# janelia-flyem/transfer_em

Hardware: AMD Instinct MI355X
Metric: CycleGAN train steps/sec on 132^3 x1 uint8 volumes (per-GPU batch of 1 volume; aggregate over GPUs) (higher is better)
Workload: dtype f32; 1 GPU; 3D 132^3 single-channel synthetic volumes, batch=1 per GPU, fp32, EM2EM.train_step (BASELINE.json configs[1]); global_batch=1, dimsize=132, parallelism=dp1

## Files before the change

transfer_em_amd/csrc/wino.hip:

```cpp
#include "tem_common.h"
#include "wino_common.h"
#include <cmath>
#include <cstdio>
#include <cstdlib>

namespace wino {

#ifdef TEM_DEBUG_KNOBS
#define KDBG(x) (x)
#else
#define KDBG(x) 0
#endif


struct Ep32 {
  float slope;
  const float *gate; int32_t gN, gD, gH, gW; float gate_slope;
  const uint8_t *keep_mask;
  int32_t doz, doy, dox, dD, dH, dW;
  int32_t gbytes, mbytes;
};

struct Dev {
  const float *in0, *in1;
  int32_t i0N, i0D, i0H, i0W, i1N, i1D, i1H, i1W;
  int32_t C0;
  int32_t N, D, H, W;
  const float *u;
  float *out0, *out1;
  int32_t o0N, o0D, o0H, o0W, o1N, o1D, o1H, o1W;
  int32_t CO0;
  int32_t OD, OH, OW;
  int32_t P;
  int32_t BY, BX, nby, nbx, zsegs, zper, NTZ;
  int32_t E, PLC, subb, slotb;
  int32_t ndma;
  int32_t span0, span1;
  uint32_t magicBX, magicE;
  int32_t dbg;
  int32_t obytes;
  unsigned long long *stamps;
  Ep32 ep;
};

template <int CI, int CO, int NI, int EP, int EE>
__global__ __launch_bounds__(512) void wino_conv_k(Dev p) {
  constexpr int NH = CI / 8, VB = 32;
  constexpr int NB = (CO + 15) / 16;
  constexpr bool STREAM = CI == 32;
  constexpr bool PAIR = CI == 8 && CO == 8;
  constexpr int NKZ = PAIR ? 4 : 3;
  constexpr int UCH = 2 * NB * 16 * 128;
  extern __shared__ __attribute__((aligned(16))) float lds[];
  char *const ring = reinterpret_cast<char *>(lds);
  const int tid = threadIdx.x, lane = tid & 63;
  const int wave = __builtin_amdgcn_readfirstlane(tid >> 6);
  const int m = lane & 15, q = lane >> 4;
  const int grp = PAIR ? wave : (NB == 1 ? wave >> 1 : wave >> 2);
  const int nb = NB == 1 ? 0 : (wave >> 1) & 1;
  const int zb = PAIR ? (q >> 1) : (wave & 1);
  const int co = PAIR ? 4 * (q & 1) : nb * 16 + 4 * q;
  float *const uld = reinterpret_cast<float *>(ring + 4 * p.slotb);

  int seg = (int)xcd_contiguous_block(blockIdx.x, gridDim.x);
  const int zseg = seg % p.zsegs; seg /= p.zsegs;
  const int bx = seg % p.nbx; seg /= p.nbx;
  const int by = seg % p.nby;
  const int n = seg / p.nby;
  const int tz0 = zseg * p.zper, tz1 = min(p.NTZ, tz0 + p.zper), nsteps = tz1 - tz0;
  const int oy0 = by * 2 * p.BY, ox0 = bx * 2 * p.BX;
  const int ntile = p.BY * p.BX;

  const bool two_in = p.in1 != p.in0;
  const float *const in0n = p.in0 + (size_t)n * p.i0N, *const in1n = p.in1 + (size_t)n * p.i1N;
  int voff0[NI], voff1[NI];
  {
    const int iy0 = oy0 - p.P, ix0 = ox0 - p.P;
#pragma unroll
    for (int i = 0; i < NI; ++i) {
      const int sp = (wave + 8 * i) * 64 + lane;
      const bool ex = sp < p.PLC;
      const int spc = ex ? sp : 0;
      const int cpos = spc & 1, ve = spc >> 1;
      const int ro = ve / EE, e = ve - ro * EE;
      const int o = ro & 1, yr = ro >> 1;
      const int c = (cpos ^ swz(e, yr)) * 4;
      const int iy = iy0 + yr, ix = ix0 + 2 * e + o;
      const bool ok = ex && (unsigned)iy < (unsigned)p.H && (unsigned)ix < (unsigned)p.W;
      voff0[i] = ok ? (iy * p.i0H + ix * p.i0W + c) * 4 : (int)0x80000000;
      voff1[i] = ok ? (iy * p.i1H + ix * p.i1W + c) * 4 : (int)0x80000000;
      asm volatile("" : "+v"(voff0[i]), "+v"(voff1[i]));
    }
  }
  auto dma_plane = [&](int iz, int slot) {
    const bool zok = (unsigned)iz < (unsigned)p.D;
    const int izc = zok ? iz : 0;
#pragma unroll
    for (int h = 0; h < NH; ++h) {
      char *const dst = ring + slot * p.slotb + h * p.subb;
      if (!two_in || 8 * h < p.C0)
        dma_subimage<NI, !STREAM>(in0n + izc * p.i0D + 8 * h, zok ? p.span0 - 32 * h : 0, voff0, dst, wave, p.ndma);
      else
        dma_subimage<NI, !STREAM>(in1n + izc * p.i1D + (8 * h - p.C0), zok ? p.span1 - 4 * (8 * h - p.C0) : 0, voff1, dst, wave, p.ndma);
    }
  };

  const int izb0 = 2 * tz0 - p.P;
  if (nsteps > 0) {
#pragma unroll
    for (int k = 0; k < 4; ++k) dma_plane(izb0 + k, k);
  }
  auto dma_u = [&](int chunk, int buf) {
    const __amdgpu_buffer_rsrc_t r = __builtin_amdgcn_make_buffer_rsrc((void *)(p.u + (size_t)chunk * UCH), 0, UCH * 4, 0x00020000);
#pragma unroll
    for (int i = 0; i < UCH * 4 / 1024 / 8; ++i) {
      const int j = wave + 8 * i;
      __builtin_amdgcn_raw_ptr_buffer_load_lds(r, (__attribute__((address_space(3))) void *)((char *)uld + buf * (UCH * 4) + j * 1024), 16,
                                               (j * 64 + lane) * 16, 0, 0, 0);
    }
  };
  if (STREAM) {
    dma_u(0, 0);
  } else {
    constexpr int UF4 = NKZ * NH * NB * 16 * 64 * 2 / 4;
    static_assert(UF4 % 512 == 0, "whole 1 KB wave transfers");
    const __amdgpu_buffer_rsrc_t ur = __builtin_amdgcn_make_buffer_rsrc((void *)p.u, 0, UF4 * 16, 0x00020000);
#pragma unroll
    for (int i = 0; i < UF4 / 512; ++i) {
      const int j = wave + 8 * i;
      __builtin_amdgcn_raw_ptr_buffer_load_lds(ur, (__attribute__((address_space(3))) void *)((char *)uld + j * 1024), 16,
                                               (j * 64 + lane) * 16, 0, 0, 0);
    }
  }
  asm volatile("s_waitcnt vmcnt(0)" ::: "memory");
  __syncthreads();

  constexpr int rowb = EE * VB;
  const Ep32 &ep = p.ep;
  float *const out0n = p.out0 + (size_t)n * p.o0N, *const out1n = EP == 2 ? p.out1 + (size_t)n * p.o1N : nullptr;
  const float *const gaten = EP >= 1 ? ep.gate + (size_t)n * ep.gN : nullptr;
  const bool in0c = EP != 2 || co < p.CO0;
  float *const obase = EP == 2 ? (in0c ? out0n : out1n) : out0n;
  const int oco = in0c ? co : co - p.CO0;
  const int oD = in0c ? p.o0D : p.o1D, oH = in0c ? p.o0H : p.o1H, oW = in0c ? p.o0W : p.o1W;
  const __amdgpu_buffer_rsrc_t grs = __builtin_amdgcn_make_buffer_rsrc((void *)gaten, 0, EP >= 1 ? ep.gbytes : 0, 0x00020000);
  const __amdgpu_buffer_rsrc_t mrs = __builtin_amdgcn_make_buffer_rsrc((void *)ep.keep_mask, 0, EP == 2 ? ep.mbytes : 0, 0x00020000);
  const int mpv = EP == 2 ? p.CO0 >> 3 : 0;
  const int kshift = co & 4;
  int gso[4], mso[4], oso[4];
#pragma unroll
  for (int o4 = 0; o4 < 4; ++o4) {
    gso[o4] = EP >= 1 ? ((o4 >> 1) * ep.gH + (o4 & 1) * ep.gW) * 4 : 0;
    mso[o4] = EP == 2 ? ((o4 >> 1) * ep.dW + (o4 & 1)) * mpv : 0;
    oso[o4] = ((o4 >> 1) * p.o0H + (o4 & 1) * p.o0W) * 4;
  }
  const __amdgpu_buffer_rsrc_t ors = __builtin_amdgcn_make_buffer_rsrc((void *)out0n, 0, EP != 2 ? p.obytes : 0, 0x00020000);

  const int tA = min(grp * 16 + m, ntile - 1);
  const int tyA = (int)fdiv((uint32_t)tA, (uint32_t)p.BX, p.magicBX), txA = tA - tyA * p.BX;
  const int a0 = (4 * tyA * EE + txA) * VB + (q & 1) * 8;
  int cs[2][2];
#pragma unroll
  for (int a = 0; a < 2; ++a)
#pragma unroll
    for (int b = 0; b < 2; ++b) cs[a][b] = ((q >> 1) ^ swz(txA + a, 2 * (tyA + b))) * 16;

#ifdef TEM_DEBUG_KNOBS
  unsigned long long t_last = p.stamps ? clock64() : 0, t_sum[8] = {0, 0, 0, 0, 0, 0, 0, 0};
#define STAMP(i) do { if (p.stamps) { unsigned long long t_now = clock64(); t_sum[i] += t_now - t_last; t_last = t_now; } } while (0)
#else
#define STAMP(i) do { } while (0)
#endif
  f32x4 acc[16];
  f32x4 gv[4];
  uint32_t kb[4];
  uint32_t tyx, tok4 = 0;
  {
    const int t = grp * 16 + m;
    const int ty = (int)fdiv((uint32_t)t, (uint32_t)p.BX, p.magicBX), tx = t - ty * p.BX;
    const int oy = oy0 + 2 * ty, ox = ox0 + 2 * tx;
    const bool tok = co < CO && t < ntile;
#pragma unroll
    for (int o4 = 0; o4 < 4; ++o4) tok4 |= ((tok && oy + (o4 >> 1) < p.OH && ox + (o4 & 1) < p.OW) ? 1u : 0u) << o4;
    tyx = ((uint32_t)oy << 16) | (uint32_t)ox;
  }
  auto tile_geom = [&](int oz, int &o0, int &go, int &mb, uint32_t &okm) {
    uint32_t yx = tyx;
    asm volatile("" : "+v"(yx));
    const int oy = (int)(yx >> 16), ox = (int)(yx & 0xffffu);
    okm = oz < p.OD ? tok4 : 0u;
    o0 = oz * oD + oy * oH + ox * oW + oco;
    go = EP >= 1 ? (oz * ep.gD + oy * ep.gH + ox * ep.gW + co) * 4 : 0;
    mb = EP == 2 ? (int)(((((uint32_t)n * ep.dD + (oz + ep.doz)) * ep.dH + (oy + ep.doy)) * ep.dW + (ox + ep.dox)) * (uint32_t)mpv) + (co >> 3) : 0;
  };
  auto fetch_ep = [&](int oz) {
    int o0, go, mb;
    uint32_t okm;
    tile_geom(oz, o0, go, mb, okm);
    if (!in0c) okm = 0;
#pragma unroll
    for (int o4 = 0; o4 < 4; ++o4) {
      const bool okf = (okm >> o4) & 1u;
      int goff = okf ? go : (int)0x80000000;
      asm volatile("" : "+v"(goff));
      const u32x4 g4 = __builtin_amdgcn_raw_buffer_load_b128(grs, goff, gso[o4], 0);
      gv[o4] = f32x4{__uint_as_float(g4.x), __uint_as_float(g4.y), __uint_as_float(g4.z), __uint_as_float(g4.w)};
      if (EP == 2) {
        int moff = okf ? mb : (int)0x80000000;
        asm volatile("" : "+v"(moff));
        kb[o4] = (uint32_t)__builtin_amdgcn_raw_buffer_load_b8(mrs, moff, mso[o4], 0) >> kshift;
      }
    }
  };
  auto finish = [&](int oz) {
    f32x4 yx[4][2], yy[2][2];
#pragma unroll
    for (int a = 0; a < 4; ++a) at4(acc[a * 4 + 0], acc[a * 4 + 1], acc[a * 4 + 2], acc[a * 4 + 3], yx[a][0], yx[a][1]);
#pragma unroll
    for (int b = 0; b < 2; ++b) at4(yx[0][b], yx[1][b], yx[2][b], yx[3][b], yy[0][b], yy[1][b]);
    int o0, go, mb;
    uint32_t okm;
    tile_geom(oz, o0, go, mb, okm);
#pragma unroll
    for (int o4 = 0; o4 < 4; ++o4) {
      const bool ok = (okm >> o4) & 1u;
      f32x4 val = yy[o4 >> 1][o4 & 1];
#pragma unroll
      for (int r = 0; r < 4; ++r) {
        if (EP == 0) val[r] = fmaxf(val[r], ep.slope * val[r]);
        if (EP >= 1 && in0c) {
          val[r] = gv[o4][r] > 0.f ? val[r] : ep.gate_slope * val[r];
          if (EP == 2) val[r] = ((kb[o4] >> r) & 1u) ? 2.f * val[r] : 0.f;
        }
      }
      if (EP == 2 || STREAM) {
        if (ok) *reinterpret_cast<f32x4 *>(obase + o0 + (o4 >> 1) * oH + (o4 & 1) * oW) = val;
      } else {
        int so = ok ? o0 * 4 + oso[o4] : (int)0x80000000;
        asm volatile("" : "+v"(so));
        __builtin_amdgcn_raw_buffer_store_b128(u32x4{__float_as_uint(val[0]), __float_as_uint(val[1]), __float_as_uint(val[2]), __float_as_uint(val[3])},
                                               ors, so, 0, 0);
      }
    }
  };

  for (int step = 0; step < nsteps; ++step) {
    const int tz = tz0 + step, oz = 2 * tz + zb, izb = 2 * tz - p.P;
    const bool more = step + 1 < nsteps;
    const int sA = (step & 1) ? 2 : 0;
    STAMP(0);
    if (EP >= 1) fetch_ep(oz);

#pragma unroll
    for (int i = 0; i < 16; ++i) acc[i] = f32x4{0.f, 0.f, 0.f, 0.f};
#pragma unroll
    for (int kz = 0; kz < NKZ; ++kz) {
      const int pl = PAIR ? kz : zb + kz;
      const char *plane = ring + ((pl < 2 ? sA : 2 - sA) + (pl & 1)) * p.slotb + a0;
#pragma unroll
      for (int h = 0; h < NH; ++h) {
        f32x2 v[4][4];
#pragma unroll
        for (int dy = 0; dy < 4; ++dy)
#pragma unroll
          for (int dx = 0; dx < 4; ++dx)
            v[dy][dx] = *reinterpret_cast<const f32x2 *>(plane + h * p.subb + (2 * dy + (dx & 1)) * rowb + (dx >> 1) * VB + cs[dx >> 1][dy >> 1]);
        if (kz == 1 && h == NH - 1) {
          __syncthreads();
          if (more && !(KDBG(p.dbg & 4))) { dma_plane(izb + 4, sA); dma_plane(izb + 5, sA + 1); }
        }
#pragma unroll
        for (int a = 0; a < 4; ++a) bt4(v[a][0], v[a][1], v[a][2], v[a][3]);
#pragma unroll
        for (int b = 0; b < 4; ++b) bt4(v[0][b], v[1][b], v[2][b], v[3][b]);
        if (STREAM && !(h & 1)) {
          const int c = kz * 2 + (h >> 1);
          if (c > 0) __syncthreads();
          if (c < 5) dma_u(c + 1, (c + 1) & 1);
          else if (more) dma_u(0, 0);
        }
        const float *uh = STREAM ? uld + ((kz * 2 + (h >> 1)) & 1) * UCH + (((h & 1) * NB + nb) * 16) * 128 + lane * 2
                                 : uld + (((kz * NH + h) * NB + nb) * 16) * 128 + lane * 2;
        f32x2 uf[16];
#pragma unroll
        for (int pt = 0; pt < 16; ++pt) uf[pt] = *reinterpret_cast<const f32x2 *>(uh + pt * 128);
#pragma unroll
        for (int pt = 0; pt < 16; ++pt) acc[pt] = __builtin_amdgcn_mfma_f32_16x16x4f32(uf[pt].x, v[pt >> 2][pt & 3].x, acc[pt], 0, 0, 0);
#pragma unroll
        for (int pt = 0; pt < 16; ++pt) acc[pt] = __builtin_amdgcn_mfma_f32_16x16x4f32(uf[pt].y, v[pt >> 2][pt & 3].y, acc[pt], 0, 0, 0);
      }
    }
    STAMP(1);

    finish(oz);
    STAMP(3);
    asm volatile("s_waitcnt vmcnt(0)" ::: "memory");
    __syncthreads();
  }
  static_assert(!PAIR || EP <= 1, "8 -> 8: forward and gated input-gradient only");

#ifdef TEM_DEBUG_KNOBS
  if (p.stamps && lane == 0) {
    for (int i = 0; i < 8; ++i) p.stamps[((size_t)blockIdx.x * 8 + wave) * 8 + i] = t_sum[i];
  }
#endif
#undef STAMP
}

__global__ __launch_bounds__(256) void wino_weights_k(const float *theta, float *u, const tem_wino_layer *layers) {
  const tem_wino_layer L = layers[blockIdx.x];
  const int nb = blockIdx.z, NB = (L.co + 15) / 16;
  const int co = nb * 16 + (threadIdx.x & 15), ci = (threadIdx.x >> 4) + 16 * blockIdx.y;
  if (ci >= L.ci || nb >= NB) return;
  const int NH = L.ci / 8;
  const bool pair = L.ci == 8 && L.co == 8;
  const int h = ci >> 3, q = (ci & 7) >> 1, j = ci & 1;
  if (pair) {
    if (nb) return;
    const int c16 = threadIdx.x & 15, s_ = c16 >> 3, c8 = c16 & 7;
    auto g4p = [](float a, float b, float c, float (&o)[4]) {
      o[0] = a; o[1] = 0.5f * (a + b + c); o[2] = 0.5f * (a - b + c); o[3] = c;
    };
    for (int pl = 0; pl < 4; ++pl) {
      const int kz = pl - s_;
      float gy[4][4];
      if (kz >= 0 && kz <= 2) {
        float g[3][3], gx[3][4];
        for (int t9 = 0; t9 < 9; ++t9) {
          const int t = kz * 9 + t9;
          g[t9 / 3][t9 % 3] = L.flip ? theta[L.src_off + ((int64_t)(26 - t) * 8 + c8) * 8 + ci] : theta[L.src_off + ((int64_t)t * 8 + ci) * 8 + c8];
        }
        for (int a = 0; a < 3; ++a) g4p(g[a][0], g[a][1], g[a][2], gx[a]);
        for (int x = 0; x < 4; ++x) {
          float o[4];
          g4p(gx[0][x], gx[1][x], gx[2][x], o);
          for (int y = 0; y < 4; ++y) gy[y][x] = o[y];
        }
      } else {
        for (int y = 0; y < 4; ++y) for (int x = 0; x < 4; ++x) gy[y][x] = 0.f;
      }
      float *d = u + L.dst_off + ((int64_t)(pl * 16) * 64 + (q * 16 + c16)) * 2 + j;
      for (int pt = 0; pt < 16; ++pt) d[pt * 128] = gy[pt >> 2][pt & 3];
    }
    return;
  }
  auto g4 = [](float a, float b, float c, float (&o)[4]) {
    o[0] = a; o[1] = 0.5f * (a + b + c); o[2] = 0.5f * (a - b + c); o[3] = c;
  };
#pragma unroll
  for (int kz = 0; kz < 3; ++kz) {
    float g[3][3];
#pragma unroll
    for (int t9 = 0; t9 < 9; ++t9) {
      const int t = kz * 9 + t9;
      float w = 0.f;
      if (co < L.co) w = L.flip ? theta[L.src_off + ((int64_t)(26 - t) * L.co + co) * L.ci + ci]
                                : theta[L.src_off + ((int64_t)t * L.ci + ci) * L.co + co];
      g[t9 / 3][t9 % 3] = w;
    }
    float gx[3][4], gy[4][4];
#pragma unroll
    for (int a = 0; a < 3; ++a) g4(g[a][0], g[a][1], g[a][2], gx[a]);
#pragma unroll
    for (int x = 0; x < 4; ++x) {
      float o[4];
      g4(gx[0][x], gx[1][x], gx[2][x], o);
#pragma unroll
      for (int y = 0; y < 4; ++y) gy[y][x] = o[y];
    }
    float *d = u + L.dst_off + ((int64_t)(((kz * NH + h) * NB + nb) * 16) * 64 + (q * 16 + (co & 15))) * 2 + j;
#pragma unroll
    for (int pt = 0; pt < 16; ++pt) d[pt * 128] = gy[pt >> 2][pt & 3];
  }
}

constexpr int LDS_MAX = 160 * 1024;

template <int CI, int CO, int NI>
int plan(Dev &p, double *cost, size_t *lds_bytes, int EE, const int32_t *pin = nullptr) {
  constexpr int NH = CI / 8, NB = (CO + 15) / 16;
  constexpr bool PAIR = CI == 8 && CO == 8;
  const size_t ubytes = CI == 32 ? (size_t)2 * (2 * NB * 16 * 128) * 4
                                 : (size_t)(PAIR ? 4 : 3) * NH * NB * 16 * 64 * 2 * 4;
  const int TY = (p.OH + 1) / 2, TX = (p.OW + 1) / 2;
  double best = 1e300;
  static const int knob_cus = tem_env_int("TEM_WINO_CUS", 256), knob_cuw = tem_env_int("TEM_WINO_CUW", 400);
  for (int by = 1; by <= TY && by <= 64; ++by)
    for (int bx = 1; bx <= TX && bx <= 64; ++bx) {
      const int nt = by * bx;
      if (nt > (PAIR ? 128 : 64 / NB)) continue;
      if (bx + 1 > EE) continue;
      if (!tem_pin_ok(pin, 1, by) || !tem_pin_ok(pin, 2, bx)) continue;
      const int E = EE, plv = (2 * by + 2) * 2 * E;
      const int subb = (plv * 32 + 1023) & ~1023, slotb = NH * subb;
      const size_t bytes = (size_t)4 * slotb + ubytes;
      const int ndma = subb / 1024;
      if (bytes > (size_t)LDS_MAX || ndma > 8 * NI) continue;
      const int nby = (TY + by - 1) / by, nbx = (TX + bx - 1) / bx;
      const int cols = p.N * nby * nbx;
      const int wraps = (16 % bx) ? 1 : 0;
      const double step = 2.0 * (PAIR ? 4 : 3) * NH * 32 * 45.0 * (1.0 + 0.03 * wraps) + 3500.0 + (CI == 32 ? 3000.0 : 0.0);
      const double pro = 6000.0 + (4.0 * slotb + ubytes) / 10.0;
      for (int zs = 1; zs <= p.NTZ; ++zs) {
        const int zper = (p.NTZ + zs - 1) / zs, zsegs = (p.NTZ + zper - 1) / zper;
        if (zsegs != zs || !tem_pin_ok(pin, 3, zsegs)) continue;
        const double t = std::ceil(cols * zsegs / (double)knob_cus) * (pro + zper * step) +
                         knob_cuw / 100.0 * (cols * zsegs / 256.0) * (pro + zper * step);
        if (t < best) {
          best = t; p.BY = by; p.BX = bx; p.nby = nby; p.nbx = nbx; p.zsegs = zsegs; p.zper = zper;
          p.E = E; p.PLC = plv * 2; p.subb = subb; p.slotb = slotb; p.ndma = ndma; *lds_bytes = (bytes + 15) & ~(size_t)15;
        }
      }
    }
  *cost = best;
  return best < 1e300 ? TEM_OK : TEM_EUNSUPPORTED;
}

template <int CI, int CO, int NI>
int plan_memo(Dev &p, double *cost, size_t *lds_bytes, int EE) {
  struct R { int rc, BY, BX, nby, nbx, zsegs, zper, E, PLC, subb, slotb, ndma; size_t lds; double cost; };
  static tem_plan_cache<5, R> cache;
  const std::array<int, 5> key{p.N, p.OH, p.OW, p.NTZ, EE};
  R r;
  if (!cache.get(key, r)) {
    r.lds = 0; r.cost = 1e300;
    r.rc = plan<CI, CO, NI>(p, &r.cost, &r.lds, EE);
    r.BY = p.BY; r.BX = p.BX; r.nby = p.nby; r.nbx = p.nbx; r.zsegs = p.zsegs; r.zper = p.zper; r.E = p.E; r.PLC = p.PLC;
    r.subb = p.subb; r.slotb = p.slotb; r.ndma = p.ndma;
    cache.put(key, r);
  } else {
    p.BY = r.BY; p.BX = r.BX; p.nby = r.nby; p.nbx = r.nbx; p.zsegs = r.zsegs; p.zper = r.zper; p.E = r.E; p.PLC = r.PLC;
    p.subb = r.subb; p.slotb = r.slotb; p.ndma = r.ndma;
  }
  *cost = r.cost; *lds_bytes = r.lds;
  return r.rc;
}

template <int CI, int CO, int NI, int EP, int EE>
static int launch(const Dev &p, size_t lds_bytes, hipStream_t st) {
  const int nblocks = p.N * p.nby * p.nbx * p.zsegs;
  auto kern = wino_conv_k<CI, CO, NI, EP, EE>;
  static bool attr_set = false;
  if (!attr_set) {
    hipError_t e = hipFuncSetAttribute((const void *)kern, hipFuncAttributeMaxDynamicSharedMemorySize, LDS_MAX);
    if (e != hipSuccess) return (int)e;
    attr_set = true;
  }
  hipLaunchKernelGGL(kern, dim3(nblocks), dim3(512), lds_bytes, st, p);
  TEM_CHECK_LAUNCH();
  return TEM_OK;
}

template <int CI, int CO, int NI, int EP>
int run_best(Dev p, hipStream_t st, bool dry, char *name, int name_len) {
  static int force = -1;
  if (force < 0) force = tem_env_int("TEM_WINO_EE", 0);
  const int pitches[2] = {9, 17};
  const int32_t *const pin = tem_plan_pinned(TEM_PLAN_WINO);
  Dev best = p;
  double cbest = 1e300;
  size_t lds_bytes = 0;
  for (int i = 0; i < 2; ++i) {
    if ((force && pitches[i] != force) || !tem_pin_ok(pin, 0, pitches[i])) continue;
    Dev q = p;
    double c = 1e300;
    size_t l = 0;
    const int rc = pin ? plan<CI, CO, NI>(q, &c, &l, pitches[i], pin) : plan_memo<CI, CO, NI>(q, &c, &l, pitches[i]);
    if (rc == TEM_OK && c < cbest) { best = q; cbest = c; lds_bytes = l; }
  }
  if (cbest >= 1e300) return TEM_EUNSUPPORTED;
  p = best;
  p.magicBX = magic_for(p.BX); p.magicE = magic_for(p.E);
  tem_plan_note(TEM_PLAN_WINO, p.E, p.BY, p.BX, p.zsegs, p.zper, p.nby, p.nbx, p.ndma);
  if (dry) {
    if (name) snprintf(name, name_len, "wino_conv_k<%d, %d, %d, %d, %d>", CI, CO, NI, EP, p.E);
    return TEM_OK;
  }
  const int nblocks = p.N * p.nby * p.nbx * p.zsegs;
  if (KDBG(p.dbg & 8))
    fprintf(stderr, "wino<%d,%d,%d> O=%dx%dx%d: BY=%d BX=%d nby=%d nbx=%d zsegs=%d zper=%d blocks=%d lds=%zu\n", CI, CO, EP,
            p.OD, p.OH, p.OW, p.BY, p.BX, p.nby, p.nbx, p.zsegs, p.zper, nblocks, lds_bytes);
  return p.E == 9 ? launch<CI, CO, NI, EP, 9>(p, lds_bytes, st) : launch<CI, CO, NI, EP, 17>(p, lds_bytes, st);
}

int dispatch(const tem_conv_args *a, hipStream_t st, bool dry, char *name, int name_len) {
  const tem_view &i0 = a->in0, &o0 = a->out0;
  const bool cube = a->kd == 3 && a->kh == 3 && a->kw == 3 && a->sd == 1 && a->sh == 1 && a->sw == 1 && a->pd == a->ph &&
                    a->ph == a->pw;
  if (!cube || a->w_layout != TEM_W_WINOGRAD || a->pd < 0) return TEM_EUNSUPPORTED;
  if (!fits32_sN(i0) || !fits32_sN(o0)) return TEM_EUNSUPPORTED;
  Dev p{};
  p.in0 = i0.ptr; p.i0N = (int)i0.sN; p.i0D = (int)i0.sD; p.i0H = (int)i0.sH; p.i0W = (int)i0.sW; p.C0 = i0.C;
  p.in1 = i0.ptr; p.i1N = p.i0N; p.i1D = p.i0D; p.i1H = p.i0H; p.i1W = p.i0W;
  int CI = i0.C;
  auto aligned = [](const tem_view &v) {
    return ((uintptr_t)v.ptr & 15) == 0 && v.sW % 4 == 0 && v.sH % 4 == 0 && v.sD % 4 == 0 && v.sN % 4 == 0 && v.C % 4 == 0;
  };
  if (!aligned(i0)) return TEM_EUNSUPPORTED;
  if (a->in1.ptr) {
    const tem_view &i1 = a->in1;
    if (i1.N != i0.N || i1.D != i0.D || i1.H != i0.H || i1.W != i0.W) return TEM_ESHAPE;
    if (!fits32_sN(i1) || !aligned(i1)) return TEM_EUNSUPPORTED;
    p.in1 = i1.ptr; p.i1N = (int)i1.sN; p.i1D = (int)i1.sD; p.i1H = (int)i1.sH; p.i1W = (int)i1.sW;
    CI += i1.C;
    if (i0.C % 8) return TEM_EUNSUPPORTED;
  }
  p.N = i0.N; p.D = i0.D; p.H = i0.H; p.W = i0.W;
  {
    const int64_t ps0 = (int64_t)(i0.H - 1) * i0.sH + (int64_t)(i0.W - 1) * i0.sW + i0.C;
    const int64_t ps1 = a->in1.ptr ? (int64_t)(i0.H - 1) * a->in1.sH + (int64_t)(i0.W - 1) * a->in1.sW + a->in1.C : 0;
    if (ps0 >= ((int64_t)1 << 29) || ps1 >= ((int64_t)1 << 29)) return TEM_EUNSUPPORTED;
  }
  p.span0 = (int)(((int64_t)(i0.H - 1) * p.i0H + (int64_t)(i0.W - 1) * p.i0W + i0.C) * 4);
  p.span1 = a->in1.ptr ? (int)(((int64_t)(i0.H - 1) * p.i1H + (int64_t)(i0.W - 1) * p.i1W + a->in1.C) * 4) : p.span0;
  p.u = a->w;
  p.out0 = o0.ptr; p.o0N = (int)o0.sN; p.o0D = (int)o0.sD; p.o0H = (int)o0.sH; p.o0W = (int)o0.sW; p.CO0 = o0.C;
  {
    const int64_t ospan = (int64_t)(o0.D - 1) * o0.sD + (int64_t)(o0.H - 1) * o0.sH + (int64_t)(o0.W - 1) * o0.sW + o0.C;
    if (ospan >= ((int64_t)1 << 29)) return TEM_EUNSUPPORTED;
    p.obytes = (int)(ospan * 4);
  }
  int CO = o0.C;
  if (a->out1.ptr) {
    const tem_view &o1 = a->out1;
    if (o1.N != o0.N || o1.D != o0.D || o1.H != o0.H || o1.W != o0.W) return TEM_ESHAPE;
    if (!fits32_sN(o1)) return TEM_EUNSUPPORTED;
    p.out1 = o1.ptr; p.o1N = (int)o1.sN; p.o1D = (int)o1.sD; p.o1H = (int)o1.sH; p.o1W = (int)o1.sW;
    CO += o1.C;
  }
  if (o0.N != i0.N) return TEM_ESHAPE;
  if (o0.D != i0.D + 2 * a->pd - 2 || o0.H != i0.H + 2 * a->ph - 2 || o0.W != i0.W + 2 * a->pw - 2) return TEM_ESHAPE;
  p.OD = o0.D; p.OH = o0.H; p.OW = o0.W;
  p.NTZ = (p.OD + 1) / 2;
  p.P = a->pd;
  {
    static int dbg = -1;
    if (dbg < 0) dbg = tem_env_int("TEM_DEBUG_FLAGS", 0);
    p.dbg = dbg;
    static unsigned long long stamp_ptr = ~0ull;
    if (stamp_ptr == ~0ull) stamp_ptr = tem_env_hex("TEM_WINO_STAMP_BUF");
    p.stamps = (unsigned long long *)stamp_ptr;
  }
  const tem_epilogue &e = a->ep;
  Ep32 &q = p.ep;
  if (e.bias || e.add.ptr) return TEM_EUNSUPPORTED;
  q.slope = e.slope; q.gate_slope = e.gate_slope;
  if (!(e.slope >= 0.f && e.slope <= 1.f)) return TEM_EUNSUPPORTED;
  int EP = 0;
  if (e.gate.ptr) {
    const tem_view &g = e.gate;
    if (g.N != o0.N || g.D != o0.D || g.H != o0.H || g.W != o0.W || g.C < o0.C) return TEM_ESHAPE;
    if (!fits32_sN(g) || e.slope != 1.f) return TEM_EUNSUPPORTED;
    q.gate = g.ptr; q.gN = (int)g.sN; q.gD = (int)g.sD; q.gH = (int)g.sH; q.gW = (int)g.sW;
    const int64_t gspan = (int64_t)(g.D - 1) * g.sD + (int64_t)(g.H - 1) * g.sH + (int64_t)(g.W - 1) * g.sW + g.C;
    if (gspan >= ((int64_t)1 << 29)) return TEM_EUNSUPPORTED;
    q.gbytes = (int)(gspan * 4);
    EP = 1;
  }
  if (e.dropout || a->out1.ptr) {
    if (!(e.dropout && e.keep_mask && e.keep_mode == 2 && a->out1.ptr && EP == 1)) return TEM_EUNSUPPORTED;
    q.keep_mask = e.keep_mask;
    q.doz = e.drop_org[0]; q.doy = e.drop_org[1]; q.dox = e.drop_org[2];
    q.dD = e.drop_dims[0] ? e.drop_dims[0] : o0.D; q.dH = e.drop_dims[0] ? e.drop_dims[1] : o0.H;
    q.dW = e.drop_dims[0] ? e.drop_dims[2] : o0.W;
    if ((int64_t)o0.N * q.dD * q.dH * q.dW * o0.C >= ((int64_t)1 << 32)) return TEM_EUNSUPPORTED;
    if (o0.C % 8) return TEM_EUNSUPPORTED;
    q.mbytes = (int)(((int64_t)o0.N * q.dD * q.dH * q.dW * o0.C + 7) / 8);
    EP = 2;
  }
#define WINO_CASE(ci, co, ni, epi) if (CI == ci && CO == co && EP == epi) return run_best<ci, co, ni, epi>(p, st, dry, name, name_len);
  WINO_CASE(16, 16, 2, 0) WINO_CASE(16, 16, 2, 1) WINO_CASE(16, 16, 2, 2)
  WINO_CASE(8, 8, 3, 0) WINO_CASE(8, 8, 3, 1)
  WINO_CASE(8, 16, 2, 0) WINO_CASE(8, 16, 2, 1)
  WINO_CASE(16, 8, 2, 0) WINO_CASE(16, 8, 2, 1)
  WINO_CASE(16, 32, 2, 0) WINO_CASE(16, 32, 2, 1)
  WINO_CASE(32, 32, 2, 0) WINO_CASE(32, 32, 2, 1) WINO_CASE(32, 32, 2, 2)
  WINO_CASE(32, 16, 2, 0) WINO_CASE(32, 16, 2, 1)
#undef WINO_CASE
  return TEM_EUNSUPPORTED;
}

}

int tem_conv_wino_try(const tem_conv_args *a, hipStream_t st, bool dry) { return wino::dispatch(a, st, dry, nullptr, 0); }

int tem_conv_wino_describe(const tem_conv_args *a, char *buf, int len) {
  int rc = wino::dispatch(a, nullptr, true, buf, len);
  return rc;
}

extern "C" int tem_winograd_weights(const float *theta, float *u, const tem_wino_layer *layers_dev, int32_t nlayers,
                                    tem_stream_t stream) {
  TEM_CLEAR_ERR();
  if (!theta || !u || !layers_dev || nlayers <= 0) return TEM_EINVAL;
  hipLaunchKernelGGL(wino::wino_weights_k, dim3(nlayers, 2, 2), dim3(256), 0, (hipStream_t)stream, theta, u, layers_dev);
  TEM_CHECK_LAUNCH();
  return TEM_OK;
}
```

transfer_em_amd/csrc/wino_common.h:

```cpp
#pragma once
#include "tem_common.h"

namespace wino {

typedef float f32x4 __attribute__((ext_vector_type(4)));
typedef float f32x2 __attribute__((ext_vector_type(2)));
typedef uint32_t u32x4 __attribute__((ext_vector_type(4)));

__device__ __forceinline__ uint32_t fdiv(uint32_t x, uint32_t d, uint32_t magic) { return d == 1 ? x : __umulhi(x, magic); }

__device__ __forceinline__ float sadd(float a, float b) { float r; asm("v_add_f32 %0, %1, %2" : "=v"(r) : "v"(a), "v"(b)); return r; }
__device__ __forceinline__ float ssub(float a, float b) { float r; asm("v_sub_f32 %0, %1, %2" : "=v"(r) : "v"(a), "v"(b)); return r; }

template <typename T> __device__ __forceinline__ void bt4(T &a, T &b, T &c, T &d) {
  const T v0 = a - c, v1 = b + c, v2 = c - b, v3 = b - d;
  a = v0; b = v1; c = v2; d = v3;
}
#ifdef TEM_WINO_SCALAR_ADDS
template <> __device__ __forceinline__ void bt4<f32x2>(f32x2 &a, f32x2 &b, f32x2 &c, f32x2 &d) {
  const f32x2 v0 = {ssub(a.x, c.x), ssub(a.y, c.y)}, v1 = {sadd(b.x, c.x), sadd(b.y, c.y)};
  const f32x2 v2 = {ssub(c.x, b.x), ssub(c.y, b.y)}, v3 = {ssub(b.x, d.x), ssub(b.y, d.y)};
  a = v0; b = v1; c = v2; d = v3;
}
#endif
template <typename T> __device__ __forceinline__ void at4(const T &a, const T &b, const T &c, const T &d, T &y0, T &y1) {
  const T s = b + c, t = b - c;
  y0 = a + s; y1 = t - d;
}

__device__ __forceinline__ int swz(int e, int yr) { return ((e >> 3) + ((yr >> 1) & 1)) & 1; }

template <int NI, bool ASM = false>
__device__ __forceinline__ void dma_subimage(const float *base, int span, const int *voff, char *dst, int wave, int ndma) {
  if constexpr (ASM) {
    typedef uint32_t u32x4_t __attribute__((ext_vector_type(4)));
    const u32x4_t r = u32x4_t{(uint32_t)__builtin_amdgcn_readfirstlane((int)(uint32_t)(uintptr_t)base),
                              (uint32_t)__builtin_amdgcn_readfirstlane((int)((uint32_t)((uintptr_t)base >> 32) & 0xffffu)), (uint32_t)span, 0x00020000u};
    const uint32_t d0 = (uint32_t)(uintptr_t)(__attribute__((address_space(3))) char *)dst;
#pragma unroll
    for (int i = 0; i < NI; ++i) {
      const int j = wave + 8 * i;
      if (j < ndma)
        asm volatile("s_mov_b32 m0, %0\n\tbuffer_load_dwordx4 %1, %2, 0 offen lds" ::"s"(d0 + j * 1024), "v"(voff[i]), "s"(r) : "memory");
    }
  } else {
    const __amdgpu_buffer_rsrc_t r = __builtin_amdgcn_make_buffer_rsrc((void *)base, 0, span, 0x00020000);
#pragma unroll
    for (int i = 0; i < NI; ++i) {
      const int j = wave + 8 * i;
      if (j < ndma)
        __builtin_amdgcn_raw_ptr_buffer_load_lds(r, (__attribute__((address_space(3))) void *)(dst + j * 1024), 16, voff[i], 0, 0, 0);
    }
  }
}

}
```

Before: 142.5 steps/s.

## Stage prologue loads per z-plane and overlap with first step compute

```diff
diff --git a/transfer_em_amd/csrc/wino.hip b/transfer_em_amd/csrc/wino.hip
--- a/transfer_em_amd/csrc/wino.hip
+++ b/transfer_em_amd/csrc/wino.hip
@@ -3,6 +3,7 @@
 #include <cmath>
 #include <cstdio>
 #include <cstdlib>
+#include <type_traits>
 
 namespace wino {
 
@@ -53,6 +54,9 @@
   constexpr int UCH = 2 * NB * 16 * 128;
   extern __shared__ __attribute__((aligned(16))) float lds[];
   char *const ring = reinterpret_cast<char *>(lds);
+#ifdef TEM_DEBUG_KNOBS
+  const unsigned long long t_begin = clock64();
+#endif
   const int tid = threadIdx.x, lane = tid & 63;
   const int wave = __builtin_amdgcn_readfirstlane(tid >> 6);
   const int m = lane & 15, q = lane >> 4;
@@ -106,10 +110,9 @@
   };
 
   const int izb0 = 2 * tz0 - p.P;
-  if (nsteps > 0) {
-#pragma unroll
-    for (int k = 0; k < 4; ++k) dma_plane(izb0 + k, k);
-  }
+  const bool oldw = KDBG(p.dbg & 512);
+  constexpr int nU = NH * NB;
+  const int nP = NH * dma_count(wave, p.ndma, NI), nG = nP + nU;
   auto dma_u = [&](int chunk, int buf) {
     const __amdgpu_buffer_rsrc_t r = __builtin_amdgcn_make_buffer_rsrc((void *)(p.u + (size_t)chunk * UCH), 0, UCH * 4, 0x00020000);
 #pragma unroll
@@ -119,21 +122,41 @@
                                                (j * 64 + lane) * 16, 0, 0, 0);
     }
   };
-  if (STREAM) {
-    dma_u(0, 0);
-  } else {
-    constexpr int UF4 = NKZ * NH * NB * 16 * 64 * 2 / 4;
-    static_assert(UF4 % 512 == 0, "whole 1 KB wave transfers");
-    const __amdgpu_buffer_rsrc_t ur = __builtin_amdgcn_make_buffer_rsrc((void *)p.u, 0, UF4 * 16, 0x00020000);
-#pragma unroll
-    for (int i = 0; i < UF4 / 512; ++i) {
+  const u32x4 ur = u32x4{(uint32_t)__builtin_amdgcn_readfirstlane((int)(uint32_t)(uintptr_t)p.u),
+                         (uint32_t)__builtin_amdgcn_readfirstlane((int)((uint32_t)((uintptr_t)p.u >> 32) & 0xffffu)),
+                         (uint32_t)(STREAM ? 0 : NKZ * nU * 8192), 0x00020000u};
+  const uint32_t ul0 = (uint32_t)(uintptr_t)(__attribute__((address_space(3))) char *)uld;
+  auto u_part = [&](int kz) {
+#pragma unroll
+    for (int i = kz * nU; i < (kz + 1) * nU; ++i) {
       const int j = wave + 8 * i;
-      __builtin_amdgcn_raw_ptr_buffer_load_lds(ur, (__attribute__((address_space(3))) void *)((char *)uld + j * 1024), 16,
-                                               (j * 64 + lane) * 16, 0, 0, 0);
-    }
-  }
-  asm volatile("s_waitcnt vmcnt(0)" ::: "memory");
-  __syncthreads();
+      dma_1k_asm(ur, (j * 64 + lane) * 16, ul0 + j * 1024);
+    }
+  };
+  auto issue_first = [&]() {
+    if constexpr (STREAM) {
+#pragma unroll
+      for (int k = 0; k < 4; ++k) dma_plane(izb0 + k, k);
+      dma_u(0, 0);
+    } else if constexpr (PAIR) {
+      dma_plane(izb0, 0); u_part(0);
+    } else {
+      dma_plane(izb0, 0); dma_plane(izb0 + 1, 1); u_part(0);
+    }
+  };
+  auto issue_rest = [&]() {
+    if constexpr (PAIR) {
+#pragma unroll
+      for (int k = 1; k < 4; ++k) { dma_plane(izb0 + k, k); u_part(k); }
+    } else if constexpr (!STREAM) {
+      dma_plane(izb0 + 2, 2); u_part(1);
+      dma_plane(izb0 + 3, 3); u_part(2);
+    }
+  };
+  if (nsteps > 0) {
+    issue_first();
+    if (EP == 0) issue_rest();
+  }
 
   constexpr int rowb = EE * VB;
   const Ep32 &ep = p.ep;
@@ -166,7 +189,7 @@
     for (int b = 0; b < 2; ++b) cs[a][b] = ((q >> 1) ^ swz(txA + a, 2 * (tyA + b))) * 16;
 
 #ifdef TEM_DEBUG_KNOBS
-  unsigned long long t_last = p.stamps ? clock64() : 0, t_sum[8] = {0, 0, 0, 0, 0, 0, 0, 0};
+  unsigned long long t_last = t_begin, t_sum[8] = {0, 0, 0, 0, 0, 0, 0, 0};
 #define STAMP(i) do { if (p.stamps) { unsigned long long t_now = clock64(); t_sum[i] += t_now - t_last; t_last = t_now; } } while (0)
 #else
 #define STAMP(i) do { } while (0)
@@ -244,12 +267,24 @@
     }
   };
 
-  for (int step = 0; step < nsteps; ++step) {
+
+  if (EP >= 1 && !STREAM && nsteps > 0) {
+    fetch_ep(2 * tz0 + zb);
+    issue_rest();
+  }
+  if (STREAM || oldw) asm volatile("s_waitcnt vmcnt(0)" ::: "memory");
+  else vm_wait((PAIR ? 3 : 2) * nG);
+  __syncthreads();
+  STAMP(5);
+
+  auto step_body = [&](auto firstc, const int step) {
+    constexpr bool FIRST = decltype(firstc)::value;
     const int tz = tz0 + step, oz = 2 * tz + zb, izb = 2 * tz - p.P;
     const bool more = step + 1 < nsteps;
     const int sA = (step & 1) ? 2 : 0;
-    STAMP(0);
-    if (EP >= 1) fetch_ep(oz);
+    const bool first = FIRST && !oldw;
+    const int nF = (more && !(KDBG(p.dbg & 4))) ? 2 * nP : 0;
+    if (EP >= 1 && (STREAM || !FIRST)) fetch_ep(oz);
 
 #pragma unroll
     for (int i = 0; i < 16; ++i) acc[i] = f32x4{0.f, 0.f, 0.f, 0.f};
@@ -260,13 +295,32 @@
 #pragma unroll
       for (int h = 0; h < NH; ++h) {
         f32x2 v[4][4];
+        if (!STREAM && !PAIR && kz == 1 && h == 0) {
+          STAMP(1);
+          if (first) vm_wait(nG);
+          else asm volatile("s_waitcnt vmcnt(0)" ::: "memory");
+          __syncthreads();
+          STAMP(0);
+        }
+        if (!STREAM && h == 0 && (PAIR ? (kz == 1 || kz == 3) : kz == 2) && first) {
+          STAMP(1);
+          vm_wait(PAIR && kz == 1 ? 2 * nG : nF);
+          __syncthreads();
+          STAMP(0);
+        }
 #pragma unroll
         for (int dy = 0; dy < 4; ++dy)
 #pragma unroll
           for (int dx = 0; dx < 4; ++dx)
             v[dy][dx] = *reinterpret_cast<const f32x2 *>(plane + h * p.subb + (2 * dy + (dx & 1)) * rowb + (dx >> 1) * VB + cs[dx >> 1][dy >> 1]);
         if (kz == 1 && h == NH - 1) {
+          if (PAIR) {
+            STAMP(1);
+            if (first) vm_wait(nG);
+            else asm volatile("s_waitcnt vmcnt(0)" ::: "memory");
+          }
           __syncthreads();
+          if (PAIR) STAMP(0);
           if (more && !(KDBG(p.dbg & 4))) { dma_plane(izb + 4, sA); dma_plane(izb + 5, sA + 1); }
         }
 #pragma unroll
@@ -294,9 +348,14 @@
 
     finish(oz);
     STAMP(3);
-    asm volatile("s_waitcnt vmcnt(0)" ::: "memory");
-    __syncthreads();
-  }
+    if (STREAM || oldw) {
+      asm volatile("s_waitcnt vmcnt(0)" ::: "memory");
+      __syncthreads();
+      STAMP(4);
+    }
+  };
+  if (!STREAM && nsteps > 0) step_body(std::true_type{}, 0);
+  for (int step = STREAM ? 0 : 1; step < nsteps; ++step) step_body(std::false_type{}, step);
   static_assert(!PAIR || EP <= 1, "8 -> 8: forward and gated input-gradient only");
 
 #ifdef TEM_DEBUG_KNOBS
diff --git a/transfer_em_amd/csrc/wino_common.h b/transfer_em_amd/csrc/wino_common.h
--- a/transfer_em_amd/csrc/wino_common.h
+++ b/transfer_em_amd/csrc/wino_common.h
@@ -30,6 +30,24 @@
 
 __device__ __forceinline__ int swz(int e, int yr) { return ((e >> 3) + ((yr >> 1) & 1)) & 1; }
 
+__device__ __forceinline__ void dma_1k_asm(u32x4 r, int voff, uint32_t lds_addr) {
+  asm volatile("s_mov_b32 m0, %0\n\tbuffer_load_dwordx4 %1, %2, 0 offen lds" ::"s"(lds_addr), "v"(voff), "s"(r) : "memory");
+}
+
+__device__ __forceinline__ int dma_count(int wave, int ndma, int ni) {
+  return __builtin_amdgcn_readfirstlane(min(ni, max(0, (ndma - wave + 7) >> 3)));
+}
+
+__device__ __forceinline__ void vm_wait(int n) {
+#define TEM_VMW(k) case k: asm volatile("s_waitcnt vmcnt(" #k ")" ::: "memory"); break;
+  switch (__builtin_amdgcn_readfirstlane(n)) {
+    TEM_VMW(1) TEM_VMW(2) TEM_VMW(3) TEM_VMW(4) TEM_VMW(5) TEM_VMW(6) TEM_VMW(7) TEM_VMW(8) TEM_VMW(9) TEM_VMW(10) TEM_VMW(11)
+    TEM_VMW(12) TEM_VMW(13) TEM_VMW(14) TEM_VMW(15) TEM_VMW(16)
+    default: asm volatile("s_waitcnt vmcnt(0)" ::: "memory"); break;
+  }
+#undef TEM_VMW
+}
+
 template <int NI, bool ASM = false>
 __device__ __forceinline__ void dma_subimage(const float *base, int span, const int *voff, char *dst, int wave, int ndma) {
   if constexpr (ASM) {
```

Measured after the change: 142.3 steps/s. Within noise of the previous version (-0.1%).
